# Arcadia-Science/arcadia-microscopy-tools

Measured on AMD Instinct MI355X. Metric: fields-of-view/sec (4x2048^2 uint16) end-to-end segment+props, higher is better.
Workload: dtype f64; 1 GPU; configs[2]: synthetic 4-channel 2048x2048 uint16 FOVs, DAPI Gaussian+Otsu+open/close+EDT+peak markers+watershed nuclei (SEEDED relief, seeds_first: marker pixels spread first in raster order, cannot tie; SURVEY A.8's plain -EDT relief with exact ties is reported under sublines.a8_exact) + clear_border/relabel + morphology and 4-channel intensity regionprops; mode=weak scaling, 192 FOVs per GPU per step, streams_per_gpu=4, fovs_per_launch=48, max_cells_per_fov=2048, distinct_fovs_per_gpu=8, resident_in_hbm=True

## Files before the change

### arcadia_microscopy_tools_amd/csrc/amt_watershed.hip

```cpp
#include "amt_internal.h"
#include <hip/hip_ext.h>

enum { CLS_NONE = 0, CLS_UNIFORM = 1, CLS_S = 3, CLS_M = 4, CLS_M2 = 5, CLS_L = 6, CLS_X = 7, CLS_G = 9 };
constexpr int WS_NLISTS = CLS_X - CLS_S + 1;
constexpr int WS_CTR = 24;
enum {
    WS_CTR_X = 0,
    WS_CTR_HBM = 7,
    WS_CTR_HASG = 8,
    WS_CTR_WL = 9,
    WS_CTR_NCOMP = 16
};
constexpr int S_PX = 2048, S_NB = 512;
constexpr int M_PX = 4096, M_NB = 512;
constexpr int M2_PX = 8192, M2_NB = 1024;
constexpr int L_PX = 24576, L_NB = 2048;
constexpr int X_PX = 32512, X_NB = 2048;
constexpr int WS_BOX_BLOCKS = 64, WS_BOX_ROWS = 32;

struct comp_row {
    int cmax;
    int mcnt;
    int x0, y0, x1, y1;
    int labmin, labmax;
    int cls;
    int root;
    int npix;
};

__global__ void __launch_bounds__(256) ws_seed_kernel(const int* __restrict__ markers, const int* __restrict__ L,
                                                      const int* __restrict__ F, int* __restrict__ out, size_t n,
                                                      const int* __restrict__ only_planes, amt_runtabs rt, int W) {
    if (only_planes && !only_planes[blockIdx.y]) return;
    const size_t base = (size_t)blockIdx.y * n;
    if (rt.tbits) {
        for (size_t i = (size_t)blockIdx.x * 256 + threadIdx.x; i < n; i += (size_t)gridDim.x * 256) {
            const long long ri = amt_rt_px_run(rt, blockIdx.y, (int)(i / W), (int)(i % W));
            int v = 0;
            if (ri >= 0) {
                const int f = F[base + amt_rt_run_root(rt, ri, W)];
                v = f > 0 ? f : (f == 0 ? markers[base + i] : 0);
// ... 45 lines not shown
        int t = 0;
        if (k < cnt) {
            t = lst[k];
            int r = L[t];
            int p = L[r];
            while (p != r) {
                r = p;
                p = L[r];
            }
            if (r != t) L[t] = r;
            else is_root = true;
        }
        const unsigned long long m = __ballot(is_root);
        if (m) {
            int base = 0;
            if (lane == __ffsll((long long)m) - 1) base = atomicAdd(&ncomp[plane], __popcll(m));
            base = __shfl(base, __ffsll((long long)m) - 1);
            if (is_root) T[t] = base + __popcll(m & ((1ull << lane) - 1ull)) + 1;
        }
    }
}

__global__ void __launch_bounds__(256) ws_rows_init_kernel(comp_row* __restrict__ rows, const int* __restrict__ ncomp,
                                                           size_t plane_stride) {
    comp_row* r = rows + (size_t)blockIdx.y * plane_stride;
    const int nc = ncomp[blockIdx.y];
    for (int i = blockIdx.x * 256 + threadIdx.x; i < nc; i += gridDim.x * 256) {
        comp_row c;
        c.cmax = 0;
        c.mcnt = 0;
        c.x0 = c.y0 = 0x7fffffff;
        c.x1 = c.y1 = -1;
        c.labmin = 0x7fffffff;
        c.labmax = 0;
        c.cls = CLS_NONE;
        c.root = -1;
        c.npix = 0;
        r[i] = c;
    }
}

template <bool MARKER_PLANE>
__global__ void __launch_bounds__(256) ws_stats_kernel(const int* __restrict__ d2, const int* __restrict__ L,
                                                       const int* __restrict__ T, const int* __restrict__ markers,
                                                       comp_row* __restrict__ rows, size_t row_stride, int H, int W,
                                                       int use_d2) {
    const int lane = threadIdx.x & 63;
// ... 432 lines not shown
            if (child >= end) break;
            int cv = a[child];
            if (child + 1 < end) {
                const int c2 = a[child + 1];
                if (c2 > cv) {
                    cv = c2;
                    ++child;
                }
            }
            if (cv <= v) break;
            a[root] = cv;
            root = child;
        }
        a[root] = v;
    };
    for (int i = n / 2 - 1; i >= 0; --i) sift(i, n, a[i]);
    for (int end = n - 1; end > 0; --end) {
        const int v = a[end];
        a[end] = a[0];
        sift(0, end, v);
    }
}

template <int TILE_PX, int NB, int CLS>
__global__ void __launch_bounds__(64) ws_flood_lds_kernel(const int* __restrict__ d2all, const int* __restrict__ Lall,
                                                          const int* __restrict__ Tall, int* __restrict__ outall,
                                                          const comp_row* __restrict__ rows,
                                                          const int* __restrict__ wl, const int* __restrict__ wl_count,
                                                          int* __restrict__ counters, size_t row_stride, int H, int W,
                                                          int seeds_first, int* __restrict__ ties,
                                                          const int* __restrict__ mkall, amt_runtabs rt) {
    extern __shared__ __attribute__((aligned(16))) char smem_raw[];
    unsigned* cell = reinterpret_cast<unsigned*>(smem_raw);
    unsigned* ht = cell + TILE_PX;
    unsigned short* half = reinterpret_cast<unsigned short*>(cell);
    const int plane = blockIdx.y;
    const size_t n = (size_t)H * W;
    const int* d2 = d2all + (size_t)plane * n;
    const int* L = Lall + (size_t)plane * n;
    const int* T = Tall + (size_t)plane * n;
    int* out = outall + (size_t)plane * n;
    const int* mk = mkall + (size_t)plane * n;
    const comp_row* rr = rows + (size_t)plane * row_stride;
    const int* mylist = wl + (size_t)plane * row_stride;
    const int nwork = wl_count[plane];
    const int lane = threadIdx.x;
    while (true) {
        int k = 0;
        if (lane == 0) k = atomicAdd(&counters[plane], 1);
        k = __builtin_amdgcn_readfirstlane(k);
        if (k >= nwork) break;
        const int c = mylist[k];
        const comp_row cr = rr[c];
        const int tw = cr.x1 - cr.x0 + 3, th = cr.y1 - cr.y0 + 3;
        const int npx = tw * th;
        const int nb = cr.cmax + 1;
        const unsigned inv_tw = 0xFFFFFFFFu / (unsigned)tw + 1u;
        for (int i0 = 0; i0 < npx; i0 += 256) {
            int rr4[4], o4[4], d4[4];
#pragma unroll
            for (int u = 0; u < 4; ++u) {
                const int i = i0 + u * 64 + lane;
                const int ty = (int)(((unsigned long long)(unsigned)i * inv_tw) >> 32), tx = i - ty * tw;
                rr4[u] = -1;
                o4[u] = 0;
// ... 99 lines not shown
                    if (cur >= 0) ht[cur] = 0xFFFFFFFFu;
                    while (cur >= 0) {
                        const int bi = cur - 1 - lane;
                        const unsigned h = bi >= 0 ? ht[bi] : 0xFFFFFFFFu;
                        const unsigned long long m = __ballot((h & 0xFFFFu) != NONE);
                        if (m) {
                            const int k = __ffsll((long long)m) - 1;
                            cur = cur - 1 - k;
                            const unsigned hk = (unsigned)__builtin_amdgcn_readlane((int)h, k);
                            head = hk & 0xFFFFu;
                            tail = hk >> 16;
                            break;
                        }
                        cur -= 64;
                    }
                    if (cur < 0) break;
                }
                spread((int)head, true);
            }
        }
        __builtin_amdgcn_wave_barrier();
        for (int i = lane; i < npx; i += 64) {
            const unsigned lv = cell[i] & 0xFFFFu;
            if (lv != 0xFFFFu) {
                const int ty = (int)(((unsigned long long)(unsigned)i * inv_tw) >> 32), tx = i - ty * tw;
                out[(size_t)(cr.y0 + ty - 1) * W + (cr.x0 + tx - 1)] = (int)lv;
            }
        }
        __builtin_amdgcn_wave_barrier();
    }
}

#ifdef WS_STATS
__device__ unsigned long long ws_dbg[8];
extern "C" int amt_ws_debug_read(unsigned long long* host8) {
    return hipMemcpyFromSymbol(host8, HIP_SYMBOL(ws_dbg), 64) == hipSuccess ? 0 : -2;
}
extern "C" int amt_ws_debug_reset() {
    unsigned long long z[8] = {0};
    return hipMemcpyToSymbol(HIP_SYMBOL(ws_dbg), z, 64) == hipSuccess ? 0 : -2;
}
#endif
__device__ __forceinline__ void ws_flood_component(unsigned* cell, unsigned* cnt, unsigned short* offs, unsigned short* queue,
                                                   const int* __restrict__ d2, const int* __restrict__ L,
                                                   const int* __restrict__ T, int* __restrict__ out,
                                                   const int* __restrict__ mk, const comp_row& cr, int c, int W,
                                                   int seeds_first, int* __restrict__ ties, int plane, int lane,
                                                   const amt_runtabs& rt) {
    auto uni = [&](unsigned v) -> unsigned { return __builtin_amdgcn_readfirstlane(v); };
    const int tw = cr.x1 - cr.x0 + 3, th = cr.y1 - cr.y0 + 3;
    const int npx = tw * th;
    const int nb = cr.cmax + 1;
#ifdef WS_STATS
    if (lane == 0) { atomicAdd(&ws_dbg[3], 1ull); atomicAdd(&ws_dbg[4], (unsigned long long)npx); atomicAdd(&ws_dbg[5], (unsigned long long)nb); }
#endif
    const unsigned inv_tw = 0xFFFFFFFFu / (unsigned)tw + 1u;
    for (int i = lane; i < nb; i += 64) cnt[i] = 0;
    __builtin_amdgcn_s_waitcnt(0);
    __builtin_amdgcn_wave_barrier();
    constexpr int SU = 6;
    for (int i0 = 0; i0 < npx; i0 += 64 * SU) {
        int rr4[SU], o4[SU], d4[SU];
        bool in4[SU];
#pragma unroll
        for (int u = 0; u < SU; ++u) {
            const int i = i0 + u * 64 + lane;
            const int ty = (int)(((unsigned long long)(unsigned)i * inv_tw) >> 32), tx = i - ty * tw;
            in4[u] = i < npx && ty >= 1 && ty < th - 1 && tx >= 1 && tx < tw - 1;
            int gy = cr.y0 + ty - 1, gx = cr.x0 + tx - 1;
            gy = gy < cr.y0 ? cr.y0 : (gy > cr.y1 ? cr.y1 : gy);
            gx = gx < cr.x0 ? cr.x0 : (gx > cr.x1 ? cr.x1 : gx);
// ... 168 lines not shown
                    found = top - 1 - (__ffsll((long long)m) - 1);
                    break;
                }
                top -= 64;
            }
            if (found < 0) break;
            cur = found;
            ht = uni(cnt[cur]);
        }
        const int hd = (int)(ht & 0xFFFFu), tl = (int)(ht >> 16);
        const int navail = tl - hd < 64 ? tl - hd : 64;
        const bool active = lane < navail;
        const int p = active ? (int)queue[hd + lane] : 0;
        const int took = step(p, active, cur, false);
        if (lane == 0) {
            const unsigned now = cnt[cur];
            cnt[cur] = (unsigned)(hd + took) | (now & 0xFFFF0000u);
        }
        __builtin_amdgcn_s_waitcnt(0);
    }
    __builtin_amdgcn_wave_barrier();
    for (int i = lane; i < npx; i += 64) {
        const unsigned lv = cell[i] & 0xFFFFu;
        if (lv != 0xFFFFu) {
            const int ty = (int)(((unsigned long long)(unsigned)i * inv_tw) >> 32), tx = i - ty * tw;
            out[(size_t)(cr.y0 + ty - 1) * W + (cr.x0 + tx - 1)] = (int)lv;
        }
    }
    __builtin_amdgcn_wave_barrier();
}

constexpr int PF_SLOT = 2560;
constexpr int PF_SLOTS = 63;
constexpr int PF_NWAVES = 10;
constexpr int PF_NCLS = 4;

__global__ void __launch_bounds__(64) ws_flood_index_kernel(const int* __restrict__ wl_count, int* __restrict__ idx,
                                                            int* __restrict__ ctl, int nplanes) {
    __shared__ int tot[PF_NCLS];
    if (threadIdx.x < PF_NCLS) {
        const int c = threadIdx.x;
        int run = 0;
        for (int p = 0; p < nplanes; ++p) {
            idx[c * (nplanes + 1) + p] = run;
            run += wl_count[c * nplanes + p];
        }
        idx[c * (nplanes + 1) + nplanes] = run;
        tot[c] = run;
    }
    __syncthreads();
    if (threadIdx.x == 0) {
        ctl[0] = 0;
        ctl[1] = 0;
        ctl[2] = tot[3] + tot[2];
        ctl[3] = tot[1] + tot[0];
    }
}

__global__ void __launch_bounds__(PF_NWAVES * 64) ws_flood_persist_kernel(
    const int* __restrict__ d2all, const int* __restrict__ Lall, const int* __restrict__ Tall, int* __restrict__ outall,
    const comp_row* __restrict__ rows, const int* __restrict__ wl, const int* __restrict__ idx, int* __restrict__ ctl,
    size_t row_stride, int H, int W, int seeds_first, int* __restrict__ ties, const int* __restrict__ mkall, int nplanes,
    amt_runtabs rt) {
    extern __shared__ __attribute__((aligned(16))) char pf_smem[];
    unsigned long long* slotmask = reinterpret_cast<unsigned long long*>(pf_smem + (size_t)PF_SLOTS * PF_SLOT);
    int* first_done = reinterpret_cast<int*>(slotmask + 1);
    const int lane = threadIdx.x & 63, wave = threadIdx.x >> 6;
    if (threadIdx.x == 0) {
        *slotmask = ~0ull << PF_SLOTS;
        *first_done = 0;
    }
    __syncthreads();
    const size_t n = (size_t)H * W;
    const int nbig = ctl[2], nsmall = ctl[3];
    int list = wave == 0 ? 0 : 1;
    bool first = true;
    int dry = 0;
    while (dry < 2) {
        int g = 0;
        if (lane == 0) g = atomicAdd(&ctl[list], 1);
        g = __builtin_amdgcn_readfirstlane(g);
        if (g >= (list == 0 ? nbig : nsmall)) {
            if (first && wave == 0 && lane == 0) __hip_atomic_store(first_done, 1, __ATOMIC_RELAXED, __HIP_MEMORY_SCOPE_WORKGROUP);
            first = false;
            ++dry;
            list ^= 1;
// ... 41 lines not shown
                if (x) {
                    const int at = __ffsll((long long)x) - 1;
                    unsigned long long expect = m;
                    if (__hip_atomic_compare_exchange_strong(slotmask, &expect, m | (want << at), __ATOMIC_RELAXED,
                                                             __ATOMIC_RELAXED, __HIP_MEMORY_SCOPE_WORKGROUP)) {
                        pos = at;
                        break;
                    }
                } else {
                    __builtin_amdgcn_s_sleep(16);
                }
            }
        }
        pos = __builtin_amdgcn_readfirstlane(pos);
        if (first && wave == 0) {
            if (lane == 0) __hip_atomic_store(first_done, 1, __ATOMIC_RELAXED, __HIP_MEMORY_SCOPE_WORKGROUP);
            first = false;
        }
        unsigned* cell = reinterpret_cast<unsigned*>(pf_smem + (size_t)pos * PF_SLOT);
        unsigned* cnt = cell + npx2;
        unsigned short* offs = reinterpret_cast<unsigned short*>(cnt + nb2);
        unsigned short* queue = offs + nb2;
        ws_flood_component(cell, cnt, offs, queue, d2all + (size_t)plane * n, Lall + (size_t)plane * n, Tall + (size_t)plane * n,
                           outall + (size_t)plane * n, mkall + (size_t)plane * n, cr, c, W, seeds_first, ties, plane, lane, rt);
        __builtin_amdgcn_s_waitcnt(0);
        if (lane == 0) {
            const unsigned long long want = need >= 64 ? ~0ull : ((1ull << need) - 1ull);
            __hip_atomic_fetch_and(slotmask, ~(want << pos), __ATOMIC_RELAXED, __HIP_MEMORY_SCOPE_WORKGROUP);
        }
    }
    if (wave == 0 && lane == 0) __hip_atomic_store(first_done, 1, __ATOMIC_RELAXED, __HIP_MEMORY_SCOPE_WORKGROUP);
}

__global__ void __launch_bounds__(64) ws_flood_edt_kernel(const int* __restrict__ d2all, const uint8_t* __restrict__ maskall,
                                                          int* __restrict__ outall, int* __restrict__ nextall,
                                                          int* __restrict__ headall, int* __restrict__ tailall,
                                                          int* __restrict__ mlistall, const comp_row* __restrict__ rows,
                                                          const int* __restrict__ moffall, const int* __restrict__ boffall,
                                                          const int* __restrict__ ncomp, int* __restrict__ counters,
                                                          size_t row_stride, int H, int W, size_t n, size_t bstride,
                                                          int seeds_first, int* __restrict__ ties) {
    const int plane = blockIdx.y;
    const size_t base = (size_t)plane * n;
    const size_t cb = (size_t)plane * row_stride;
    const int* d2 = d2all + base;
    const uint8_t* mask = maskall + base;
    int* out = outall + base;
// ... 432 lines not shown
                if (fx == 0 || fy == 0 || fz == 0 || fw == 0) w = *reinterpret_cast<const int4*>(ws + base + i0);
                const int vx = fx > 0 ? fx : (fx == 0 ? w.x : 0), vy = fy > 0 ? fy : (fy == 0 ? w.y : 0);
                const int vz = fz > 0 ? fz : (fz == 0 ? w.z : 0), vw = fw > 0 ? fw : (fw == 0 ? w.w : 0);
                o.x = (unsigned)(vx - 1) < ml ? M[vx] : 0;
                o.y = (unsigned)(vy - 1) < ml ? M[vy] : 0;
                o.z = (unsigned)(vz - 1) < ml ? M[vz] : 0;
                o.w = (unsigned)(vw - 1) < ml ? M[vw] : 0;
            }
            *reinterpret_cast<int4*>(out + base + i0) = o;
        } else {
            for (size_t i = i0; i < n && i < i0 + 4; ++i) {
                const int v = ws_pixel_label(L[base + i], F, ws, base, i);
                out[base + i] = (unsigned)(v - 1) < ml ? M[v] : 0;
            }
        }
    }
}

struct ws_box_args {
    int* bbox;
    const comp_row* rows;
    const int* ncomp;
    size_t row_stride;
    int2* flist;
    int* fcount;
    int* fbig;
};

__global__ void __launch_bounds__(1024) ws_label_map_kernel(const int* __restrict__ L, const int* __restrict__ F,
                                                            const int* __restrict__ ws, int* __restrict__ present,
                                                            const int* __restrict__ nlabels, int* __restrict__ count_dev,
                                                            int H, int W, int max_label, amt_runtabs rt, ws_box_args bx) {
    __shared__ int s[1024];
    __shared__ int carry;
    __shared__ int nwalk, big;
    const int plane = blockIdx.x;
    const size_t n = (size_t)H * W;
    const size_t base = (size_t)plane * n;
    int* P = present + (size_t)plane * (max_label + 1);
    const int k = nlabels[plane] < max_label ? nlabels[plane] : max_label;
    for (int l = threadIdx.x; l <= max_label; l += 1024) P[l] = (l >= 1 && l <= k) ? 1 : 0;
    __syncthreads();
    const int perim = 2 * W + 2 * H;
    for (int q = threadIdx.x; q < perim; q += 1024) {
        int y, x;
        if (q < W) {
            y = 0;
            x = q;
        } else if (q < 2 * W) {
            y = H - 1;
            x = q - W;
        } else if (q < 2 * W + H) {
            y = q - 2 * W;
            x = 0;
        } else {
            y = q - 2 * W - H;
            x = W - 1;
        }
// ... 12 lines not shown
    __syncthreads();
    for (int start = 1; start <= max_label; start += 1024) {
        const int i = start + threadIdx.x;
        const int v = i <= max_label ? P[i] : 0;
        s[threadIdx.x] = v;
        __syncthreads();
        for (int off = 1; off < 1024; off <<= 1) {
            const int t = threadIdx.x >= off ? s[threadIdx.x - off] : 0;
            __syncthreads();
            s[threadIdx.x] += t;
            __syncthreads();
        }
        const int incl = s[threadIdx.x];
        const int c = carry;
        if (i <= max_label) P[i] = v ? c + incl : 0;
        __syncthreads();
        if (threadIdx.x == 1023) carry = c + incl;
        __syncthreads();
    }
    if (threadIdx.x == 0) count_dev[plane] = carry;
    if (!bx.bbox) return;
    int* B = bx.bbox + (size_t)plane * max_label * 4;
    for (int i = threadIdx.x; i < max_label * 4; i += 1024) B[i] = (i & 2) ? -1 : 0x7fffffff;
    if (threadIdx.x == 0) nwalk = 0, big = 0;
    __syncthreads();
    const comp_row* rows = bx.rows + (size_t)plane * bx.row_stride;
    const int fcap = (int)(bx.row_stride / 2);
    int2* fl = bx.flist + (size_t)plane * fcap;
    const int nc = bx.ncomp[plane];
    for (int i = threadIdx.x; i < nc; i += 1024) {
        const comp_row c = rows[i];
        if (c.cls == CLS_UNIFORM) {
            const int m = (unsigned)(c.labmin - 1) < (unsigned)max_label ? P[c.labmin] : 0;
            if (m > 0) {
                int* b = B + (size_t)(m - 1) * 4;
                atomicMin(&b[0], c.y0);
                atomicMin(&b[1], c.x0);
                atomicMax(&b[2], c.y1);
                atomicMax(&b[3], c.x1);
            }
        } else if (c.cls >= CLS_S) {
            const long long area = (long long)(c.x1 - c.x0 + 3) * (c.y1 - c.y0 + 3);
            const int nb = (c.y1 - c.y0) / WS_BOX_ROWS + 1, nch = (c.x1 - c.x0) / 64 + 1;
            const int at = area > X_PX ? fcap : atomicAdd(&nwalk, nb * nch);
            if (area > X_PX || at > fcap - nb * nch) {
                big = 1;
            } else {
                for (int k = 0; k < nb * nch; ++k) fl[at + k] = make_int2(i, (k % nb) | ((k / nb) << 16));
            }
        }
    }
    __syncthreads();
    if (threadIdx.x == 0) bx.fcount[plane] = big ? 0 : nwalk, bx.fbig[plane] = big;
}

__global__ void __launch_bounds__(256) ws_flood_boxes_kernel(const int* __restrict__ labels, ws_box_args bx, int H, int W,
                                                             int max_label) {
    const int lane = threadIdx.x & 63;
    const int plane = blockIdx.y;
    const int cnt = bx.fcount[plane];
    const int* Lp = labels + (size_t)plane * H * W;
    int* B = bx.bbox + (size_t)plane * max_label * 4;
    const comp_row* rows = bx.rows + (size_t)plane * bx.row_stride;
    const int2* fl = bx.flist + (size_t)plane * (bx.row_stride / 2);
    const unsigned ml = (unsigned)max_label;
    constexpr int FQ = 4;
    for (int j = blockIdx.x * 4 + (threadIdx.x >> 6); j < cnt; j += gridDim.x * 4) {
        const int2 it = fl[j];
        const comp_row c = rows[it.x];
        const int ya = c.y0 + (it.y & 0xffff) * WS_BOX_ROWS;
        const int yb = ya + WS_BOX_ROWS - 1 < c.y1 ? ya + WS_BOX_ROWS - 1 : c.y1;
        const int x = c.x0 + (it.y >> 16) * 64 + lane;
        const bool in = x <= c.x1;
        const int xl = in ? x : c.x1;
        auto load = [&](int y) -> int {
            int v = 0;
            if (in && y >= 0 && y < H && y <= yb + 1) v = Lp[(size_t)y * W + xl];
            return (unsigned)(v - 1) < ml ? v : 0;
        };
        int up = load(ya - 1), cur = load(ya);
        for (int y = ya; y <= yb; y += FQ) {
            int nx[FQ];
#pragma unroll
            for (int q = 0; q < FQ; ++q) nx[q] = load(y + 1 + q);
#pragma unroll
            for (int q = 0; q < FQ; ++q) {
                const int yy = y + q;
                if (yy > yb) break;
                const int dn = nx[q];
                const int l = amt_lane_left(cur), r = amt_lane_right(cur);
                const int ul = amt_lane_left(up), ur = amt_lane_right(up);
                const int dl = amt_lane_left(dn), dr = amt_lane_right(dn);
                if (cur) {
                    int* b = B + (size_t)(cur - 1) * 4;
                    const bool head = l != cur, tail = r != cur;
                    if (head && up != cur) atomicMin(&b[0], yy);
                    if (head && dn != cur) atomicMax(&b[2], yy);
                    if (head && ul != cur && dl != cur) atomicMin(&b[1], x);
                    if (tail && ur != cur && dr != cur) atomicMax(&b[3], x);
                }
                up = cur;
                cur = dn;
            }
        }
    }
}

__global__ void __launch_bounds__(256) ws_final_map_kernel(int* __restrict__ Fall, const int* __restrict__ map,
                                                           const int* __restrict__ rootlist, const int* __restrict__ nroots,
                                                           size_t cap, size_t n, int max_label) {
    const int plane = blockIdx.z, shard = plane * gridDim.y + blockIdx.y;
    int* F = Fall + (size_t)plane * n;
    const int* M = map + (size_t)plane * (max_label + 1);
    const int cnt = nroots[shard] < (int)cap ? nroots[shard] : (int)cap;
    const int* lst = rootlist + (size_t)shard * cap;
    for (int k = blockIdx.x * 256 + threadIdx.x; k < cnt; k += gridDim.x * 256) {
        const int t = lst[k], f = F[t];
        F[t] = f > 0 ? ((unsigned)(f - 1) < (unsigned)max_label ? M[f] : 0) : (f == 0 ? -1 : 0);
    }
}

__global__ void __launch_bounds__(256) ws_final_runs_kernel(const unsigned long long* __restrict__ tbits,
                                                            const unsigned short* __restrict__ rtab,
                                                            const int* __restrict__ nruns, const int* __restrict__ Fall,
                                                            const int* __restrict__ wsall, const int* __restrict__ map,
                                                            int* __restrict__ outall, int H, int W, int segs, int trows,
// ... 90 lines not shown
    int max_label = 0;
    const int32_t* mk_list = nullptr;
    const int32_t* mk_count = nullptr;
    int mk_cap = 0;
};

struct ws_args {
    amt_ctx* ctx;
    const void* relief;
    bool use_d2;
    const int32_t* markers;
    const uint8_t* mask;
    int32_t* out;
    int nplanes, H, W, seeds_first;
    ws_fused fu;
    ccl_geom g;
    size_t n, row_stride, bstride;
    bool runs;
};
struct ws_bufs {
    int *L, *T, *moff, *boff, *cursor, *mlist, *next, *F, *rootlist, *nroots;
    comp_row* rows;
    int *btot, *mtot, *counters, *wl, *pf_idx, *pf_ctl, *ccl_scratch, *ties, *P;
    int* fctl;
    unsigned long long* tbits;
    unsigned short* rtab;
    int* nruns;
    unsigned short* roff;
    int *rcomp, *head, *tail;
    hp_elem *gheap, *heap;
    int *ncomp, *has_g, *wl_count;
    amt_runtabs rt;
};

static int ws_emulate(amt_ctx* ctx, const void* relief, bool use_d2, const int32_t* markers, const uint8_t* mask, int32_t* out,
                      hp_elem* gheap, const int* run, int nplanes, int H, int W, int conn) {
    const size_t n = (size_t)H * W;
    hipLaunchKernelGGL(ws_global_init_kernel, dim3(amt_grid_for(n, 256, 1024), nplanes), dim3(256), 0, ctx->stream, markers,
                       mask, out, run, n);
    AMT_LAUNCH_CHECK();
    amt_with_bool(use_d2, [&](auto D2) {
        hipLaunchKernelGGL((ws_global_kernel<decltype(D2)::value>), dim3(nplanes), dim3(64), GH_LDS_N * sizeof(gh_elem),
                           ctx->stream, relief, mask, out, gheap, run, H, W, n, conn);
    });
    AMT_LAUNCH_CHECK();
    return AMT_OK;
}

static int ws_label_and_classify(const ws_args& a, const ws_bufs& b) {
    amt_ctx* ctx = a.ctx;
    const ccl_geom& g = a.g;
    const int nplanes = a.nplanes, H = a.H, W = a.W;
    hipLaunchKernelGGL(ws_init_kernel, dim3(16), dim3(256), 0, ctx->stream, b.counters, nplanes * WS_CTR, b.ties, nplanes,
                       b.nroots, (int)g.nlist);
    AMT_LAUNCH_CHECK();
    if (a.runs) AMT_TRY(amt_i_ccl_tileroots_runs_u8(ctx, g, a.mask, b.L, b.rootlist, b.nroots, b.tbits, b.rtab, b.nruns, b.roff));
    else AMT_TRY(amt_i_ccl_tileroots_u8(ctx, g, a.mask, b.L, b.rootlist, b.nroots, b.ccl_scratch));
    hipLaunchKernelGGL(ws_roots_kernel, g.glists, dim3(256), 0, ctx->stream, b.L, b.T, b.rootlist, b.nroots, b.ncomp, g.cap, a.n);
    AMT_LAUNCH_CHECK();
    AMT_TRY(amt_i_propagate_roots(ctx, g, b.T, b.L, b.rootlist, b.nroots));
    hipLaunchKernelGGL(ws_rows_init_kernel, dim3(64, nplanes), dim3(256), 0, ctx->stream, b.rows, b.ncomp, a.row_stride);
    AMT_LAUNCH_CHECK();
    if (a.runs) {
        hipLaunchKernelGGL(ws_stats_runs_kernel, dim3((unsigned)((g.ntiles + 3) / 4)), dim3(256), 0, ctx->stream,
                           (const int*)a.relief, b.tbits, b.rtab, b.nruns, b.L, b.T, b.rows, a.row_stride, H, W, g.segs, g.trows,
                           (int)g.ntiles, b.rcomp);
    } else {
        amt_with_bool(!a.fu.mk_list, [&](auto MARKER_PLANE) {
            hipLaunchKernelGGL((ws_stats_kernel<decltype(MARKER_PLANE)::value>), dim3((W + 63) / 64, (H + 31) / 32, nplanes),
                               dim3(256), 0, ctx->stream, a.use_d2 ? (const int*)a.relief : (const int*)nullptr, b.L, b.T,
                               a.markers, b.rows, a.row_stride, H, W, a.use_d2 ? 1 : 0);
        });
    }
    AMT_LAUNCH_CHECK();
    if (a.fu.mk_list) {
        hipLaunchKernelGGL(ws_marker_stats_kernel, dim3(16, nplanes), dim3(256), 0, ctx->stream, a.fu.mk_list, a.fu.mk_count,
                           a.fu.mk_cap, a.markers, b.L, b.T, b.rows, a.row_stride, a.n, b.rt, W);
        AMT_LAUNCH_CHECK();
    }
    hipLaunchKernelGGL(ws_classify_kernel, dim3(64, nplanes), dim3(256), 0, ctx->stream, b.rows, b.ncomp, b.moff, b.boff, b.has_g,
                       b.wl, b.wl_count, b.F, a.n, nplanes, a.row_stride, a.use_d2 ? 1 : 0);
    AMT_LAUNCH_CHECK();
    return amt_i_propagate_roots(ctx, g, b.F, b.L, b.rootlist, b.nroots);
}
// ... 19 lines not shown
    AMT_LAUNCH_CHECK();
    hipLaunchKernelGGL(ws_fill_markers_kernel, g1, dim3(256), 0, ctx->stream, b.L, b.T, a.out, b.rows, b.moff, b.cursor, b.mlist,
                       b.has_g, a.row_stride, a.n, b.rt, a.W);
    AMT_LAUNCH_CHECK();
    if (a.use_d2) {
        hipLaunchKernelGGL(ws_fill_value_kernel, dim3(256, nplanes), dim3(256), 0, ctx->stream, b.head, b.btot, a.bstride, -1);
        AMT_LAUNCH_CHECK();
    }
    return AMT_OK;
}

static int ws_floods_d2(const ws_args& a, const ws_bufs& b) {
    amt_ctx* ctx = a.ctx;
    const int nplanes = a.nplanes;
    const size_t ldsX = (size_t)X_PX * 4 + (size_t)X_NB * 4;
    AMT_TRY(amt_fork(ctx));
    const int any = ctx->fork == 0 ? (int)hipExtAnyOrderLaunch : 0;
    hipLaunchKernelGGL(ws_flood_index_kernel, dim3(1), dim3(64), 0, ctx->stream, b.wl_count, b.pf_idx, b.pf_ctl, nplanes);
    AMT_LAUNCH_CHECK();
    const int* a_d2 = (const int*)a.relief;
    {
        void* args[] = {&a_d2, (void*)&b.L, (void*)&b.T, (void*)&a.out, (void*)&b.rows, (void*)&b.wl, (void*)&b.pf_idx,
                        (void*)&b.pf_ctl, (void*)&a.row_stride, (void*)&a.H, (void*)&a.W, (void*)&a.seeds_first, (void*)&b.ties,
                        (void*)&a.markers, (void*)&a.nplanes, (void*)&b.rt};
        AMT_HIP_CHECK(hipExtLaunchKernel((const void*)ws_flood_persist_kernel, dim3(ctx->num_cus), dim3(PF_NWAVES * 64), args,
                                         (size_t)(PF_SLOTS + 1) * PF_SLOT, ctx->stream, nullptr, nullptr, 0));
    }
    {
        const int* a_wl = b.wl + (size_t)(CLS_X - CLS_S) * nplanes * a.row_stride;
        const int* a_wlc = b.wl_count + (CLS_X - CLS_S) * nplanes;
        int* a_cnt = b.counters + WS_CTR_X * nplanes;
        void* args[] = {&a_d2, (void*)&b.L, (void*)&b.T, (void*)&a.out, (void*)&b.rows, &a_wl, &a_wlc, &a_cnt,
                        (void*)&a.row_stride, (void*)&a.H, (void*)&a.W, (void*)&a.seeds_first, (void*)&b.ties, (void*)&a.markers,
                        (void*)&b.rt};
        AMT_HIP_CHECK(hipExtLaunchKernel((const void*)ws_flood_lds_kernel<X_PX, X_NB, CLS_X>, dim3(8, nplanes), dim3(64), args,
                                         ldsX, ctx->stream, nullptr, nullptr, any));
    }
    {
        int* a_cnt = b.counters + WS_CTR_HBM * nplanes;
        void* args[] = {&a_d2, (void*)&a.mask, (void*)&a.out, (void*)&b.next, (void*)&b.head, (void*)&b.tail, (void*)&b.mlist,
                        (void*)&b.rows, (void*)&b.moff, (void*)&b.boff, (void*)&b.ncomp, &a_cnt, (void*)&a.row_stride, (void*)&a.H,
                        (void*)&a.W, (void*)&a.n, (void*)&a.bstride, (void*)&a.seeds_first, (void*)&b.ties};
        AMT_HIP_CHECK(hipExtLaunchKernel((const void*)ws_flood_edt_kernel, dim3(4, nplanes), dim3(64), args, 0, ctx->aux[1],
                                         nullptr, nullptr, any));
    }
    AMT_TRY(amt_join(ctx));
    AMT_LAUNCH_CHECK();
    return AMT_OK;
}

static int ws_flood_f64(const ws_args& a, const ws_bufs& b) {
    amt_ctx* ctx = a.ctx;
    hipLaunchKernelGGL(ws_flood_heap_kernel, dim3(64, a.nplanes), dim3(64), 0, ctx->stream, (const double*)a.relief, a.mask,
                       a.out, b.heap, b.mlist, b.rows, b.moff, b.boff, b.ncomp, b.counters + WS_CTR_HBM * a.nplanes,
                       a.row_stride, a.H, a.W, a.n, a.bstride, b.ties);
    AMT_LAUNCH_CHECK();
    return AMT_OK;
}

static int ws_fused_tail(const ws_args& a, const ws_bufs& b) {
    amt_ctx* ctx = a.ctx;
    const ccl_geom& g = a.g;
    const ws_fused& fu = a.fu;
    ws_box_args bx = {};
    if (a.runs && fu.max_label > 0 && ctx->own_stream) {
        AMT_TRY(amt_box_buffer(ctx, (size_t)a.nplanes * fu.max_label * 4, &bx.bbox));
        bx.rows = b.rows, bx.ncomp = b.ncomp, bx.row_stride = a.row_stride;
        bx.flist = reinterpret_cast<int2*>(b.cursor), bx.fcount = b.fctl, bx.fbig = b.fctl + a.nplanes;
    }
    hipLaunchKernelGGL(ws_label_map_kernel, dim3(a.nplanes), dim3(1024), 0, ctx->stream, b.L, b.F, a.out, b.P, fu.nlabels_dev,
                       fu.count, a.H, a.W, fu.max_label, b.rt, bx);
    AMT_LAUNCH_CHECK();
    if (a.runs) {
        hipLaunchKernelGGL(ws_final_map_kernel, g.glists, dim3(256), 0, ctx->stream, b.F, b.P, b.rootlist, b.nroots, g.cap, a.n,
                           fu.max_label);
        AMT_LAUNCH_CHECK();
        hipLaunchKernelGGL(ws_final_runs_kernel, dim3((unsigned)((g.ntiles + 3) / 4)), dim3(256), 0, ctx->stream, b.tbits, b.rtab,
                           b.nruns, b.F, a.out, b.P, fu.labels, a.H, a.W, g.segs, g.trows, (int)g.ntiles, fu.max_label);
        if (bx.bbox) {
            AMT_LAUNCH_CHECK();
            hipLaunchKernelGGL(ws_flood_boxes_kernel, dim3(WS_BOX_BLOCKS, a.nplanes), dim3(256), 0, ctx->stream,
                               (const int*)fu.labels, bx, a.H, a.W, fu.max_label);
            AMT_LAUNCH_CHECK();
            AMT_TRY(amt_i_label_boxes_flagged(ctx, fu.labels, bx.bbox, bx.fbig, a.nplanes, a.H, a.W, fu.max_label));
            amt_box_note_leave(ctx, fu.labels, a.nplanes, a.H, a.W, fu.max_label);
        }
    } else {
        hipLaunchKernelGGL(ws_final_kernel, dim3(amt_grid_for(a.n, 1024, 4096), a.nplanes), dim3(256), 0, ctx->stream, b.L, b.F,
                           a.out, b.P, fu.labels, a.n, fu.max_label);
    }
    AMT_LAUNCH_CHECK();
    return AMT_OK;
}

static int watershed_components(amt_ctx* ctx, const void* relief, bool use_d2, const int32_t* markers, const uint8_t* mask,
                                int32_t* out, int nplanes, int H, int W, int seeds_first, bool exact, int32_t* ties_dev,
                                const ws_fused& fu) {
    ws_args a = {ctx, relief, use_d2, markers, mask, out, nplanes, H, W, seeds_first, fu, amt_i_ccl_geom(nplanes, H, W)};
    const ccl_geom& g = a.g;
    const size_t n = a.n = g.n;
    const size_t np = (size_t)nplanes * n;
    const size_t row_stride = n / 2 + 1;
    const size_t nr = (size_t)nplanes * row_stride;
    const size_t bstride = use_d2 ? n + row_stride : n;
    a.row_stride = row_stride, a.bstride = bstride;
// ... 6 lines not shown
    amt_buf<int> moff(s, nr);
    amt_buf<int> boff(s, nr);
    amt_buf<int> cursor(s, nr);
    amt_buf<int> mlist(s, np);
    amt_buf<int> next(s, np);
    amt_buf<int> F(s, np);
    amt_buf<int> rootlist(s, g.nlist * g.cap);
    amt_buf<int> nroots(s, g.nlist);
    amt_buf<comp_row> rows(s, nr);
    amt_buf<int> btot(s, nplanes);
    amt_buf<int> mtot(s, nplanes);
    amt_buf<int> counters(s, (size_t)nplanes * WS_CTR);
    amt_buf<int> wl(s, (size_t)WS_NLISTS * nr);
    amt_buf<int> pf_idx(s, (size_t)PF_NCLS * (nplanes + 1));
    amt_buf<int> pf_ctl(s, 16);
    amt_buf<int> ccl_scratch(s, g.multi_ints());
    amt_buf<int> ties_own(s, nplanes, !ties_dev);
    amt_buf<int> P(s, (size_t)nplanes * ((size_t)fu.max_label + 1), fu.labels != nullptr);
    amt_buf<unsigned long long> tbits(s, g.ntiles * 64, runs);
    amt_buf<unsigned short> rtab(s, g.ntiles * RT_CAP, runs);
    amt_buf<int> nruns(s, g.ntiles, runs);
    amt_buf<unsigned short> roff(s, g.ntiles * 64, runs);
    amt_buf<int> rcomp(s, g.ntiles * RT_CAP, runs);
    amt_buf<int> fctl(s, (size_t)2 * nplanes, runs);
    amt_buf<int> head(s, (size_t)nplanes * bstride, use_d2);
    amt_buf<int> tail(s, (size_t)nplanes * bstride, use_d2);
    amt_buf<hp_elem> gheap_own(s, np, use_d2 && exact);
    amt_buf<hp_elem> heap(s, (size_t)nplanes * bstride, !use_d2);
    AMT_TRY(s.commit());
    ws_bufs b = {};
    b.L = L, b.T = T, b.moff = moff, b.boff = boff, b.cursor = cursor, b.mlist = mlist, b.next = next, b.F = F;
    b.rootlist = rootlist, b.nroots = nroots, b.rows = rows, b.btot = btot, b.mtot = mtot, b.counters = counters, b.wl = wl;
    b.pf_idx = pf_idx, b.pf_ctl = pf_ctl, b.ccl_scratch = ccl_scratch, b.P = P;
    b.tbits = tbits, b.rtab = rtab, b.nruns = nruns, b.roff = roff, b.rcomp = rcomp, b.head = head, b.tail = tail;
    b.fctl = fctl;
    b.ties = ties_dev ? ties_dev : ties_own.p;
    b.heap = heap, b.gheap = use_d2 ? gheap_own.p : heap.p;
    b.ncomp = b.counters + WS_CTR_NCOMP * (size_t)nplanes;
    b.has_g = b.counters + WS_CTR_HASG * nplanes;
    b.wl_count = b.counters + WS_CTR_WL * nplanes;
    b.rt = {tbits, roff, rtab, rcomp, g.segs, g.trows};

    AMT_TRY(ws_label_and_classify(a, b));
    AMT_TRY(ws_prepare_hbm(a, b, fu.labels && use_d2));
    AMT_TRY(use_d2 ? ws_floods_d2(a, b) : ws_flood_f64(a, b));
    if (exact) AMT_TRY(ws_emulate(ctx, relief, use_d2, markers, mask, out, b.gheap, b.ties, nplanes, H, W, 1));
    if (fu.labels) AMT_TRY(ws_fused_tail(a, b));
    return AMT_OK;
}

static int watershed_common(amt_ctx* ctx, const void* relief, bool use_d2, const int32_t* markers,
                            const uint8_t* mask, int32_t* out, int nplanes, int H, int W, int seeds_first,
                            int connectivity, int tie_policy, int32_t* ties_dev, const ws_fused& fu) {
    AMT_TRY(amt_set_device(ctx));
    AMT_REQUIRE(relief && markers && mask && out && nplanes >= 0 && H > 0 && W > 0, "watershed: bad arguments");
    AMT_REQUIRE((size_t)H * W < 0x3fffffffull, "watershed: plane too large");
    AMT_REQUIRE(connectivity == 1 || connectivity == 2, "watershed: connectivity must be 1 or 2, got %d", connectivity);
    AMT_REQUIRE(tie_policy == AMT_WS_TIES_EXACT || tie_policy == AMT_WS_TIES_RASTER || tie_policy == AMT_WS_TIES_REPORT,
// ... 62 lines not shown
```

Before: 17380 FOV/s.

## Compute label bounding boxes inside watershed flood kernels instead of separate pass

Removes the separate ws_flood_boxes_kernel, which re-read the final label image to find per-label bounding-box extremes. The extremes are now computed in the LDS flood kernels' write-back loop, using neighbour checks on the tile and atomics into a per-plane mbox array. The label-map kernel then folds mbox into bbox through the relabel map P. This drops a global-memory pass and a kernel launch, but adds eight LDS reads per pixel and global atomics to the flood write-back. It also makes the fbig fallback depend on has_g.

```diff
diff --git a/arcadia_microscopy_tools_amd/csrc/amt_watershed.hip b/arcadia_microscopy_tools_amd/csrc/amt_watershed.hip
--- a/arcadia_microscopy_tools_amd/csrc/amt_watershed.hip
+++ b/arcadia_microscopy_tools_amd/csrc/amt_watershed.hip
@@ -16,7 +16,6 @@
 constexpr int M2_PX = 8192, M2_NB = 1024;
 constexpr int L_PX = 24576, L_NB = 2048;
 constexpr int X_PX = 32512, X_NB = 2048;
-constexpr int WS_BOX_BLOCKS = 64, WS_BOX_ROWS = 32;
 
 struct comp_row {
     int cmax;
@@ -108,7 +107,12 @@
 }
 
 __global__ void __launch_bounds__(256) ws_rows_init_kernel(comp_row* __restrict__ rows, const int* __restrict__ ncomp,
-                                                           size_t plane_stride) {
+                                                           size_t plane_stride, int4* __restrict__ mbox, int max_label) {
+    if (mbox) {
+        int4* mb = mbox + (size_t)blockIdx.y * max_label;
+        for (int i = blockIdx.x * 256 + threadIdx.x; i < max_label; i += gridDim.x * 256)
+            mb[i] = make_int4(0x7fffffff, 0x7fffffff, -1, -1);
+    }
     comp_row* r = rows + (size_t)blockIdx.y * plane_stride;
     const int nc = ncomp[blockIdx.y];
     for (int i = blockIdx.x * 256 + threadIdx.x; i < nc; i += gridDim.x * 256) {
@@ -587,6 +591,27 @@
     }
 }
 
+__device__ __forceinline__ void ws_ask_boxes(const unsigned* cell, int i, int tw, unsigned lv, int gy, int gx,
+                                             int* __restrict__ mbox, int max_label) {
+    const unsigned v = lv != 0xFFFFu && lv - 1u < (unsigned)max_label ? lv : 0u;
+    const int ia = v ? i : tw + 1;
+    const unsigned cl = (cell[ia - 1] & 0xFFFFu) ^ v, cr = (cell[ia + 1] & 0xFFFFu) ^ v;
+    const unsigned uu = (cell[ia - tw] & 0xFFFFu) ^ v, dd = (cell[ia + tw] & 0xFFFFu) ^ v;
+    const unsigned ul = (cell[ia - tw - 1] & 0xFFFFu) ^ v, ur = (cell[ia - tw + 1] & 0xFFFFu) ^ v;
+    const unsigned dl = (cell[ia + tw - 1] & 0xFFFFu) ^ v, dr = (cell[ia + tw + 1] & 0xFFFFu) ^ v;
+    const unsigned q0 = min(min(v, cl), uu);
+    const unsigned q2 = min(min(v, cl), dd);
+    const unsigned q1 = min(min(min(cl, ul), dl), v);
+    const unsigned q3 = min(min(min(cr, ur), dr), v);
+    if (q0 | q1 | q2 | q3) {
+        int* b = mbox + (size_t)(v - 1u) * 4;
+        if (q0) atomicMin(&b[0], gy);
+        if (q2) atomicMax(&b[2], gy);
+        if (q1) atomicMin(&b[1], gx);
+        if (q3) atomicMax(&b[3], gx);
+    }
+}
+
 template <int TILE_PX, int NB, int CLS>
 __global__ void __launch_bounds__(64) ws_flood_lds_kernel(const int* __restrict__ d2all, const int* __restrict__ Lall,
                                                           const int* __restrict__ Tall, int* __restrict__ outall,
@@ -594,7 +619,8 @@
                                                           const int* __restrict__ wl, const int* __restrict__ wl_count,
                                                           int* __restrict__ counters, size_t row_stride, int H, int W,
                                                           int seeds_first, int* __restrict__ ties,
-                                                          const int* __restrict__ mkall, amt_runtabs rt) {
+                                                          const int* __restrict__ mkall, amt_runtabs rt,
+                                                          int* __restrict__ mboxall, int max_label) {
     extern __shared__ __attribute__((aligned(16))) char smem_raw[];
     unsigned* cell = reinterpret_cast<unsigned*>(smem_raw);
     unsigned* ht = cell + TILE_PX;
@@ -606,6 +632,7 @@
     const int* T = Tall + (size_t)plane * n;
     int* out = outall + (size_t)plane * n;
     const int* mk = mkall + (size_t)plane * n;
+    int* mbox = mboxall ? mboxall + (size_t)plane * max_label * 4 : nullptr;
     const comp_row* rr = rows + (size_t)plane * row_stride;
     const int* mylist = wl + (size_t)plane * row_stride;
     const int nwork = wl_count[plane];
@@ -751,10 +778,10 @@
         __builtin_amdgcn_wave_barrier();
         for (int i = lane; i < npx; i += 64) {
             const unsigned lv = cell[i] & 0xFFFFu;
-            if (lv != 0xFFFFu) {
-                const int ty = (int)(((unsigned long long)(unsigned)i * inv_tw) >> 32), tx = i - ty * tw;
-                out[(size_t)(cr.y0 + ty - 1) * W + (cr.x0 + tx - 1)] = (int)lv;
-            }
+            const int ty = (int)(((unsigned long long)(unsigned)i * inv_tw) >> 32), tx = i - ty * tw;
+            const int gy = cr.y0 + ty - 1, gx = cr.x0 + tx - 1;
+            if (lv != 0xFFFFu) out[(size_t)gy * W + gx] = (int)lv;
+            if (mbox) ws_ask_boxes(cell, i, tw, lv, gy, gx, mbox, max_label);
         }
         __builtin_amdgcn_wave_barrier();
     }
@@ -775,7 +802,7 @@
                                                    const int* __restrict__ T, int* __restrict__ out,
                                                    const int* __restrict__ mk, const comp_row& cr, int c, int W,
                                                    int seeds_first, int* __restrict__ ties, int plane, int lane,
-                                                   const amt_runtabs& rt) {
+                                                   const amt_runtabs& rt, int* __restrict__ mbox, int max_label) {
     auto uni = [&](unsigned v) -> unsigned { return __builtin_amdgcn_readfirstlane(v); };
     const int tw = cr.x1 - cr.x0 + 3, th = cr.y1 - cr.y0 + 3;
     const int npx = tw * th;
@@ -990,10 +1017,10 @@
     __builtin_amdgcn_wave_barrier();
     for (int i = lane; i < npx; i += 64) {
         const unsigned lv = cell[i] & 0xFFFFu;
-        if (lv != 0xFFFFu) {
-            const int ty = (int)(((unsigned long long)(unsigned)i * inv_tw) >> 32), tx = i - ty * tw;
-            out[(size_t)(cr.y0 + ty - 1) * W + (cr.x0 + tx - 1)] = (int)lv;
-        }
+        const int ty = (int)(((unsigned long long)(unsigned)i * inv_tw) >> 32), tx = i - ty * tw;
+        const int gy = cr.y0 + ty - 1, gx = cr.x0 + tx - 1;
+        if (lv != 0xFFFFu) out[(size_t)gy * W + gx] = (int)lv;
+        if (mbox) ws_ask_boxes(cell, i, tw, lv, gy, gx, mbox, max_label);
     }
     __builtin_amdgcn_wave_barrier();
 }
@@ -1029,7 +1056,7 @@
     const int* __restrict__ d2all, const int* __restrict__ Lall, const int* __restrict__ Tall, int* __restrict__ outall,
     const comp_row* __restrict__ rows, const int* __restrict__ wl, const int* __restrict__ idx, int* __restrict__ ctl,
     size_t row_stride, int H, int W, int seeds_first, int* __restrict__ ties, const int* __restrict__ mkall, int nplanes,
-    amt_runtabs rt) {
+    amt_runtabs rt, int* __restrict__ mboxall, int max_label) {
     extern __shared__ __attribute__((aligned(16))) char pf_smem[];
     unsigned long long* slotmask = reinterpret_cast<unsigned long long*>(pf_smem + (size_t)PF_SLOTS * PF_SLOT);
     int* first_done = reinterpret_cast<int*>(slotmask + 1);
@@ -1117,7 +1144,8 @@
         unsigned short* offs = reinterpret_cast<unsigned short*>(cnt + nb2);
         unsigned short* queue = offs + nb2;
         ws_flood_component(cell, cnt, offs, queue, d2all + (size_t)plane * n, Lall + (size_t)plane * n, Tall + (size_t)plane * n,
-                           outall + (size_t)plane * n, mkall + (size_t)plane * n, cr, c, W, seeds_first, ties, plane, lane, rt);
+                           outall + (size_t)plane * n, mkall + (size_t)plane * n, cr, c, W, seeds_first, ties, plane, lane, rt,
+                           mboxall ? mboxall + (size_t)plane * max_label * 4 : nullptr, max_label);
         __builtin_amdgcn_s_waitcnt(0);
         if (lane == 0) {
             const unsigned long long want = need >= 64 ? ~0ull : ((1ull << need) - 1ull);
@@ -1596,9 +1624,8 @@
     const comp_row* rows;
     const int* ncomp;
     size_t row_stride;
-    int2* flist;
-    int* fcount;
-    int* fbig;
+    int* mbox;
+    const int* fbig;
 };
 
 __global__ void __launch_bounds__(1024) ws_label_map_kernel(const int* __restrict__ L, const int* __restrict__ F,
@@ -1607,7 +1634,6 @@
                                                             int H, int W, int max_label, amt_runtabs rt, ws_box_args bx) {
     __shared__ int s[1024];
     __shared__ int carry;
-    __shared__ int nwalk, big;
     const int plane = blockIdx.x;
     const size_t n = (size_t)H * W;
     const size_t base = (size_t)plane * n;
@@ -1666,86 +1692,31 @@
     if (!bx.bbox) return;
     int* B = bx.bbox + (size_t)plane * max_label * 4;
     for (int i = threadIdx.x; i < max_label * 4; i += 1024) B[i] = (i & 2) ? -1 : 0x7fffffff;
-    if (threadIdx.x == 0) nwalk = 0, big = 0;
     __syncthreads();
     const comp_row* rows = bx.rows + (size_t)plane * bx.row_stride;
-    const int fcap = (int)(bx.row_stride / 2);
-    int2* fl = bx.flist + (size_t)plane * fcap;
     const int nc = bx.ncomp[plane];
     for (int i = threadIdx.x; i < nc; i += 1024) {
         const comp_row c = rows[i];
-        if (c.cls == CLS_UNIFORM) {
-            const int m = (unsigned)(c.labmin - 1) < (unsigned)max_label ? P[c.labmin] : 0;
-            if (m > 0) {
-                int* b = B + (size_t)(m - 1) * 4;
-                atomicMin(&b[0], c.y0);
-                atomicMin(&b[1], c.x0);
-                atomicMax(&b[2], c.y1);
-                atomicMax(&b[3], c.x1);
-            }
-        } else if (c.cls >= CLS_S) {
-            const long long area = (long long)(c.x1 - c.x0 + 3) * (c.y1 - c.y0 + 3);
-            const int nb = (c.y1 - c.y0) / WS_BOX_ROWS + 1, nch = (c.x1 - c.x0) / 64 + 1;
-            const int at = area > X_PX ? fcap : atomicAdd(&nwalk, nb * nch);
-            if (area > X_PX || at > fcap - nb * nch) {
-                big = 1;
-            } else {
-                for (int k = 0; k < nb * nch; ++k) fl[at + k] = make_int2(i, (k % nb) | ((k / nb) << 16));
-            }
-        }
-    }
-    __syncthreads();
-    if (threadIdx.x == 0) bx.fcount[plane] = big ? 0 : nwalk, bx.fbig[plane] = big;
-}
-
-__global__ void __launch_bounds__(256) ws_flood_boxes_kernel(const int* __restrict__ labels, ws_box_args bx, int H, int W,
-                                                             int max_label) {
-    const int lane = threadIdx.x & 63;
-    const int plane = blockIdx.y;
-    const int cnt = bx.fcount[plane];
-    const int* Lp = labels + (size_t)plane * H * W;
-    int* B = bx.bbox + (size_t)plane * max_label * 4;
-    const comp_row* rows = bx.rows + (size_t)plane * bx.row_stride;
-    const int2* fl = bx.flist + (size_t)plane * (bx.row_stride / 2);
-    const unsigned ml = (unsigned)max_label;
-    constexpr int FQ = 4;
-    for (int j = blockIdx.x * 4 + (threadIdx.x >> 6); j < cnt; j += gridDim.x * 4) {
-        const int2 it = fl[j];
-        const comp_row c = rows[it.x];
-        const int ya = c.y0 + (it.y & 0xffff) * WS_BOX_ROWS;
-        const int yb = ya + WS_BOX_ROWS - 1 < c.y1 ? ya + WS_BOX_ROWS - 1 : c.y1;
-        const int x = c.x0 + (it.y >> 16) * 64 + lane;
-        const bool in = x <= c.x1;
-        const int xl = in ? x : c.x1;
-        auto load = [&](int y) -> int {
-            int v = 0;
-            if (in && y >= 0 && y < H && y <= yb + 1) v = Lp[(size_t)y * W + xl];
-            return (unsigned)(v - 1) < ml ? v : 0;
-        };
-        int up = load(ya - 1), cur = load(ya);
-        for (int y = ya; y <= yb; y += FQ) {
-            int nx[FQ];
-#pragma unroll
-            for (int q = 0; q < FQ; ++q) nx[q] = load(y + 1 + q);
-#pragma unroll
-            for (int q = 0; q < FQ; ++q) {
-                const int yy = y + q;
-                if (yy > yb) break;
-                const int dn = nx[q];
-                const int l = amt_lane_left(cur), r = amt_lane_right(cur);
-                const int ul = amt_lane_left(up), ur = amt_lane_right(up);
-                const int dl = amt_lane_left(dn), dr = amt_lane_right(dn);
-                if (cur) {
-                    int* b = B + (size_t)(cur - 1) * 4;
-                    const bool head = l != cur, tail = r != cur;
-                    if (head && up != cur) atomicMin(&b[0], yy);
-                    if (head && dn != cur) atomicMax(&b[2], yy);
-                    if (head && ul != cur && dl != cur) atomicMin(&b[1], x);
-                    if (tail && ur != cur && dr != cur) atomicMax(&b[3], x);
-                }
-                up = cur;
-                cur = dn;
-            }
+        if (c.cls != CLS_UNIFORM) continue;
+        const int m = (unsigned)(c.labmin - 1) < (unsigned)max_label ? P[c.labmin] : 0;
+        if (m > 0) {
+            int* b = B + (size_t)(m - 1) * 4;
+            atomicMin(&b[0], c.y0);
+            atomicMin(&b[1], c.x0);
+            atomicMax(&b[2], c.y1);
+            atomicMax(&b[3], c.x1);
+        }
+    }
+    const int4* MB = reinterpret_cast<const int4*>(bx.mbox) + (size_t)plane * max_label;
+    for (int l = 1 + threadIdx.x; l <= k; l += 1024) {
+        const int m = P[l];
+        const int4 e = MB[l - 1];
+        if (m > 0 && e.z >= 0) {
+            int* b = B + (size_t)(m - 1) * 4;
+            atomicMin(&b[0], e.x);
+            atomicMin(&b[1], e.y);
+            atomicMax(&b[2], e.z);
+            atomicMax(&b[3], e.w);
         }
     }
 }
@@ -1882,7 +1853,7 @@
     int *L, *T, *moff, *boff, *cursor, *mlist, *next, *F, *rootlist, *nroots;
     comp_row* rows;
     int *btot, *mtot, *counters, *wl, *pf_idx, *pf_ctl, *ccl_scratch, *ties, *P;
-    int* fctl;
+    int* mbox;
     unsigned long long* tbits;
     unsigned short* rtab;
     int* nruns;
@@ -1919,7 +1890,8 @@
     hipLaunchKernelGGL(ws_roots_kernel, g.glists, dim3(256), 0, ctx->stream, b.L, b.T, b.rootlist, b.nroots, b.ncomp, g.cap, a.n);
     AMT_LAUNCH_CHECK();
     AMT_TRY(amt_i_propagate_roots(ctx, g, b.T, b.L, b.rootlist, b.nroots));
-    hipLaunchKernelGGL(ws_rows_init_kernel, dim3(64, nplanes), dim3(256), 0, ctx->stream, b.rows, b.ncomp, a.row_stride);
+    hipLaunchKernelGGL(ws_rows_init_kernel, dim3(64, nplanes), dim3(256), 0, ctx->stream, b.rows, b.ncomp, a.row_stride,
+                       reinterpret_cast<int4*>(b.mbox), a.fu.max_label);
     AMT_LAUNCH_CHECK();
     if (a.runs) {
         hipLaunchKernelGGL(ws_stats_runs_kernel, dim3((unsigned)((g.ntiles + 3) / 4)), dim3(256), 0, ctx->stream,
@@ -1985,7 +1957,7 @@
     {
         void* args[] = {&a_d2, (void*)&b.L, (void*)&b.T, (void*)&a.out, (void*)&b.rows, (void*)&b.wl, (void*)&b.pf_idx,
                         (void*)&b.pf_ctl, (void*)&a.row_stride, (void*)&a.H, (void*)&a.W, (void*)&a.seeds_first, (void*)&b.ties,
-                        (void*)&a.markers, (void*)&a.nplanes, (void*)&b.rt};
+                        (void*)&a.markers, (void*)&a.nplanes, (void*)&b.rt, (void*)&b.mbox, (void*)&a.fu.max_label};
         AMT_HIP_CHECK(hipExtLaunchKernel((const void*)ws_flood_persist_kernel, dim3(ctx->num_cus), dim3(PF_NWAVES * 64), args,
                                          (size_t)(PF_SLOTS + 1) * PF_SLOT, ctx->stream, nullptr, nullptr, 0));
     }
@@ -1995,7 +1967,7 @@
         int* a_cnt = b.counters + WS_CTR_X * nplanes;
         void* args[] = {&a_d2, (void*)&b.L, (void*)&b.T, (void*)&a.out, (void*)&b.rows, &a_wl, &a_wlc, &a_cnt,
                         (void*)&a.row_stride, (void*)&a.H, (void*)&a.W, (void*)&a.seeds_first, (void*)&b.ties, (void*)&a.markers,
-                        (void*)&b.rt};
+                        (void*)&b.rt, (void*)&b.mbox, (void*)&a.fu.max_label};
         AMT_HIP_CHECK(hipExtLaunchKernel((const void*)ws_flood_lds_kernel<X_PX, X_NB, CLS_X>, dim3(8, nplanes), dim3(64), args,
                                          ldsX, ctx->stream, nullptr, nullptr, any));
     }
@@ -2026,10 +1998,10 @@
     const ccl_geom& g = a.g;
     const ws_fused& fu = a.fu;
     ws_box_args bx = {};
-    if (a.runs && fu.max_label > 0 && ctx->own_stream) {
+    if (b.mbox) {
         AMT_TRY(amt_box_buffer(ctx, (size_t)a.nplanes * fu.max_label * 4, &bx.bbox));
         bx.rows = b.rows, bx.ncomp = b.ncomp, bx.row_stride = a.row_stride;
-        bx.flist = reinterpret_cast<int2*>(b.cursor), bx.fcount = b.fctl, bx.fbig = b.fctl + a.nplanes;
+        bx.mbox = b.mbox, bx.fbig = b.has_g;
     }
     hipLaunchKernelGGL(ws_label_map_kernel, dim3(a.nplanes), dim3(1024), 0, ctx->stream, b.L, b.F, a.out, b.P, fu.nlabels_dev,
                        fu.count, a.H, a.W, fu.max_label, b.rt, bx);
@@ -2041,9 +2013,6 @@
         hipLaunchKernelGGL(ws_final_runs_kernel, dim3((unsigned)((g.ntiles + 3) / 4)), dim3(256), 0, ctx->stream, b.tbits, b.rtab,
                            b.nruns, b.F, a.out, b.P, fu.labels, a.H, a.W, g.segs, g.trows, (int)g.ntiles, fu.max_label);
         if (bx.bbox) {
-            AMT_LAUNCH_CHECK();
-            hipLaunchKernelGGL(ws_flood_boxes_kernel, dim3(WS_BOX_BLOCKS, a.nplanes), dim3(256), 0, ctx->stream,
-                               (const int*)fu.labels, bx, a.H, a.W, fu.max_label);
             AMT_LAUNCH_CHECK();
             AMT_TRY(amt_i_label_boxes_flagged(ctx, fu.labels, bx.bbox, bx.fbig, a.nplanes, a.H, a.W, fu.max_label));
             amt_box_note_leave(ctx, fu.labels, a.nplanes, a.H, a.W, fu.max_label);
@@ -2096,7 +2065,7 @@
     amt_buf<int> nruns(s, g.ntiles, runs);
     amt_buf<unsigned short> roff(s, g.ntiles * 64, runs);
     amt_buf<int> rcomp(s, g.ntiles * RT_CAP, runs);
-    amt_buf<int> fctl(s, (size_t)2 * nplanes, runs);
+    amt_buf<int> mbox(s, (size_t)nplanes * fu.max_label * 4, runs && fu.max_label > 0 && ctx->own_stream);
     amt_buf<int> head(s, (size_t)nplanes * bstride, use_d2);
     amt_buf<int> tail(s, (size_t)nplanes * bstride, use_d2);
     amt_buf<hp_elem> gheap_own(s, np, use_d2 && exact);
@@ -2107,7 +2076,7 @@
     b.rootlist = rootlist, b.nroots = nroots, b.rows = rows, b.btot = btot, b.mtot = mtot, b.counters = counters, b.wl = wl;
     b.pf_idx = pf_idx, b.pf_ctl = pf_ctl, b.ccl_scratch = ccl_scratch, b.P = P;
     b.tbits = tbits, b.rtab = rtab, b.nruns = nruns, b.roff = roff, b.rcomp = rcomp, b.head = head, b.tail = tail;
-    b.fctl = fctl;
+    b.mbox = mbox;
     b.ties = ties_dev ? ties_dev : ties_own.p;
     b.heap = heap, b.gheap = use_d2 ? gheap_own.p : heap.p;
     b.ncomp = b.counters + WS_CTR_NCOMP * (size_t)nplanes;
```

New measurement: 17650 FOV/s (median of 6 runs). 1.5% higher.
